# TheCacophonyProject/classifier-pipeline

Measured on AMD Instinct MI355X. Metric: CPTV frames/s end-to-end (track+classify) at 160x120, higher is better.
Workload: dtype u16/i32 track stage (f32 normalise, f64 gates); f32 crop/tile; f32 CNN (stride-1 3x3 convs of stages 2-4 (+ the stride-2 one): two fp16 planes per operand rounded to nearest (11 + 11 significand bits), power-of-two range scaling, 3 fp16 MFMAs per K step, device-side rerun in the exact split if an ac

## Files before the change

### classifier-pipeline_amd/csrc/cpx_cnn_bf3.hip

```cpp
#include <hip/hip_runtime.h>

#include <algorithm>
#include <cstdlib>
#include <type_traits>

#include "cpx_conv_layout_core.h"
#include "cpx_kernels.h"

namespace cpx {

namespace {

typedef float f32x16 __attribute__((ext_vector_type(16)));
typedef __bf16 bf16x8 __attribute__((ext_vector_type(8)));
typedef __bf16 bf16x2 __attribute__((ext_vector_type(2)));
typedef unsigned u32x4 __attribute__((ext_vector_type(4)));
typedef float f32x4 __attribute__((ext_vector_type(4)));

__device__ __forceinline__ unsigned pack2(float a, float b) {
  bf16x2 v = {(__bf16)a, (__bf16)b};
  return __builtin_bit_cast(unsigned, v);
}
template <typename T>
__device__ __forceinline__ const T* at_off(const T* base, unsigned bytes) {
// ... 1938 lines not shown
    return launch_bf3w(a, im, w, s);
  }
  if (a.Cout / a.groups == 32) return launch_bf3_t<1, 1, NB_S2, TW_S2, CT_S2>(a, w, s);
  if (a.Cout / a.groups == 64) return launch_bf3_t<NTN_S3, 1, NB_S3, TW_S3, CT_S3>(a, w, s);
  if (flat_pays(a, 32, 4 * NB_S4, 256)) {
    if (a.planes == 2 && a.half && a.sc_in && a.sc_planes && conv_shortcut_planes_layer(a, a.sc_cin / a.groups) && !a.residual &&
        a.sc_stride >= 1 && a.sc_xscale > 0.0f && (a.sc_H - 1) / a.sc_stride + 1 == a.Ho && (a.sc_W - 1) / a.sc_stride + 1 == a.Wo &&
        (long long)a.sc_H * a.sc_W * a.sc_cin < (1ll << 31))
      return launch_bf3flat_t<2, 256, 2, true, 256, true>(a, w + im.half / 16, s);
    return with_math(a, im, w, [&](auto pl, auto h, const uint4* wi) {
      return launch_bf3flat_t<2, 256, decltype(pl)::value, decltype(h)::value>(a, wi, s);
    });
  }
  return with_math(a, im, w, [&](auto pl, auto h, const uint4* wi) {
    return launch_bf3_t<NTN_S4, 1, NB_S4, 32, CT_S4, false, decltype(pl)::value, decltype(h)::value>(a, wi, s);
  });
}

bool conv_block32_supported(const ConvArgs& a, const ConvArgs& b) {
  const auto plain = [](const ConvArgs& c) {
    return c.ksize == 3 && c.stride == 1 && c.Cout / c.groups == 32 && c.relu && c.pad_top == 1 && c.pad_left == 1 && !c.out_planes &&
           !c.in_planes;
  };
  if (!(plain(a) && plain(b) && a.in_scale && a.in_shift && !a.residual && !a.sc_in && !b.in_scale && !b.out_scale &&
        a.Cout == b.Cin && b.Cin == b.Cout && a.groups == b.groups && a.H == b.H && a.W == b.W && a.N == b.N && a.ovf != nullptr))
    return false;
  if (a.Cin / a.groups == 8)
    return b.residual == nullptr && b.sc_in == a.in && b.sc_w != nullptr && b.sc_cin == a.Cin && b.sc_stride == 1 && b.sc_H == a.H &&
           b.sc_W == a.W;
  return a.Cin == a.Cout && b.residual == a.in && b.sc_in == nullptr;
}
int launch_conv_block32(const ConvArgs& a_in, const ConvArgs& b_in, const void* wimg_a, const void* wimg_b, hipStream_t s) {
  ConvArgs a = a_in, b = b_in;
  if (!conv_block32_supported(a, b)) return -2;
  if ((long long)a.H * a.W >= (1 << 24)) return -3;
  const WeightImages ia = images_of(a), ib = images_of(b);
  if (ia.half == WeightImages::absent || ib.half == WeightImages::absent) return -2;
  a.w_scale = conv_bf3_weight_scales(a, wimg_a);
  a.w_unscale = a.w_scale + a.Cout;
  b.w_scale = conv_bf3_weight_scales(b, wimg_b);
  b.w_unscale = b.w_scale + b.Cout;
  const uint4* wa = reinterpret_cast<const uint4*>(wimg_a) + ia.half / 16;
  const uint4* wb = reinterpret_cast<const uint4*>(wimg_b) + ib.half / 16;
  TileDiv td{};
  if (const int rc = fill_tiles(td, (a.W + W_TW - 1) / W_TW, (a.H + W_TH - 1) / W_TH, a.N, 1, TILES_PERSISTENT)) return rc;
  const bool c8 = a.Cin / a.groups == 8;
  static const bool split_roles = [] {
    const char* e = std::getenv("CPX_BLOCK32_SPLIT");
    return e == nullptr || std::atoi(e) != 0;
  }();
  if (!c8 && split_roles) return launch_conv_block32s(a, b, wa, wb, s);
  const bool c1 = c8 && a.c1_in != nullptr;
  if (c1 && !(a.groups == 2 && a.c1_w != nullptr && a.c1_b != nullptr)) return -2;
  const size_t lds = c8 ? (size_t)(B_R0 + B8_WIMG + B_WIMG) * 16 + 256 + (size_t)2 * B8_NPXP * 16 + (c1 ? (size_t)(B_C1W + 2 * B_C1C) * 4 : 0)
                        : (size_t)(B_R0 + 2 * B_WIMG) * 16 + 256;
  static bool lds_ready[64], lds_ready8[64], lds_ready1[64];
  if (c1 ? !cpx_dyn_lds_ready(reinterpret_cast<const void*>(conv_block32_kernel<true, true>), lds_ready1, 160 * 1024 - 1024)
      : c8 ? !cpx_dyn_lds_ready(reinterpret_cast<const void*>(conv_block32_kernel<true>), lds_ready8, 160 * 1024 - 1024)
           : !cpx_dyn_lds_ready(reinterpret_cast<const void*>(conv_block32_kernel<false>), lds_ready, 160 * 1024 - 1024))
    return -1;
  const int cus = cpx_device_cus();
  if (cus == 0) return -1;
  const char* e = std::getenv("CPX_BLOCK32_GRID");
  const int gx = e ? persistent_grid_x(std::atoi(e), 1, td.total) : persistent_grid_x(cus, a.groups, td.total);
  if (c1) hipLaunchKernelGGL((conv_block32_kernel<true, true>), dim3((unsigned)gx, a.groups), dim3(512), lds, s, a, b, wa, wb, td);
  else if (c8) hipLaunchKernelGGL(conv_block32_kernel<true>, dim3((unsigned)gx, a.groups), dim3(512), lds, s, a, b, wa, wb, td);
  else hipLaunchKernelGGL(conv_block32_kernel<false>, dim3((unsigned)gx, a.groups), dim3(512), lds, s, a, b, wa, wb, td);
  return 0;
}

}
```

### classifier-pipeline_amd/csrc/cpx_cnn_blk.hip

```cpp
#include <hip/hip_runtime.h>

#include <algorithm>
#include <cstdlib>
#include <type_traits>

#include "cpx_conv_layout_core.h"
#include "cpx_kernels.h"

namespace cpx {

namespace {

typedef unsigned u32x4 __attribute__((ext_vector_type(4)));
typedef float f32x4 __attribute__((ext_vector_type(4)));
typedef _Float16 f16x2 __attribute__((ext_vector_type(2)));
typedef _Float16 f16x8 __attribute__((ext_vector_type(8)));

template <typename T>
__device__ __forceinline__ const T* at_off(const T* base, unsigned bytes) {
  return reinterpret_cast<const T*>(reinterpret_cast<const char*>(base) + bytes);
}
template <typename T>
__device__ __forceinline__ T* at_off(T* base, unsigned bytes) {
  return reinterpret_cast<T*>(reinterpret_cast<char*>(base) + bytes);
}
__device__ __forceinline__ unsigned pix_off(int y, int x, int W, int C) {
  return __umul24(__umul24((unsigned)y, (unsigned)W) + (unsigned)x, (unsigned)C);
}
__device__ __forceinline__ float relu_bits(float x) { return __int_as_float(max(__float_as_int(x), 0)); }
__device__ __forceinline__ void split_h(float a, float b, unsigned& hi, unsigned& lo) {
  f16x2 v = {(_Float16)a, (_Float16)b};
  hi = __builtin_bit_cast(unsigned, v);
  asm("v_fma_mixlo_f16 %0, %1, 1.0, -%2 op_sel:[0,0,0] op_sel_hi:[0,0,1]" : "=v"(lo) : "v"(a), "v"(hi));
  asm("v_fma_mixhi_f16 %0, %1, 1.0, -%2 op_sel:[0,0,1] op_sel_hi:[0,0,1]" : "+v"(lo) : "v"(b), "v"(hi));
}
__device__ __forceinline__ f32x4 mfma_h(u32x4 w, u32x4 x, f32x4 c) {
  return __builtin_amdgcn_mfma_f32_16x16x32_f16(__builtin_bit_cast(f16x8, w), __builtin_bit_cast(f16x8, x), c, 0, 0, 0);
}
__device__ __forceinline__ unsigned pk_max_u16(unsigned x, unsigned y) {
  unsigned r;
  asm("v_pk_max_u16 %0, %1, %2" : "=v"(r) : "v"(x), "v"(y));
  return r;
}
__device__ __forceinline__ int med3(int x, int lo, int hi) {
  int r;
  asm("v_med3_i32 %0, %1, %2, %3" : "=v"(r) : "v"(x), "v"(lo), "s"(hi));
  return r;
}
template <int I, int N, typename F>
__device__ __forceinline__ void static_for(F&& f) {
  if constexpr (I < N) {
    f(std::integral_constant<int, I>{});
    static_for<I + 1, N>(f);
  }
}
struct BlkTiles {
  unsigned long long m_tx, m_ty;
  int tiles_x, tiles_y, total;
};
__device__ __forceinline__ int div_magic(int n, unsigned long long m) { return (int)(((unsigned long long)n * m) >> 42); }

constexpr int K_T = 16;
constexpr int K_PP = 20, K_PNPX = 400;
constexpr int K_PNPXP = 402;
constexpr int K_MP = 18;
constexpr int K_MNPXP = 326;
constexpr int K_PBUF = 2 * 2 * K_PNPXP * 2;
constexpr int K_MBUF = 2 * 2 * K_MNPXP * 2;
constexpr int K_CT = 512;
constexpr int K_NP = 7;
constexpr int K_PPI = K_CT / 8;
constexpr int K_WROW = 2 * 3 * 4 * 32;
constexpr int K_WIMG = 3 * K_WROW;
constexpr size_t K_LDS = (size_t)(K_PBUF + 2 * K_MBUF) * 16;

__global__ __launch_bounds__(K_CT) __attribute__((amdgpu_waves_per_eu(2, 2))) void conv_block32s_kernel(ConvArgs a, ConvArgs b, const uint4* __restrict__ wa, const uint4* __restrict__ wb, BlkTiles td) {
  if (*a.ovf != 0) return;
  extern __shared__ __attribute__((aligned(16))) uint4 lds4[];
  uint4* s_P = lds4;
  uint4* s_M = lds4 + K_PBUF;
  const int tid = threadIdx.x, lane = tid & 63, wave = tid >> 6, i16 = lane & 15, q = lane >> 4;
  const bool is_a = wave < 4;
  const int ct = wave & 1, hh = (wave >> 1) & 1;
  const int g = blockIdx.y;
  const int C = b.Cout, H = a.H, W = a.W;

  u32x4 Wr[9][2];
  {
    const u32x4* wg = reinterpret_cast<const u32x4*>(is_a ? wa : wb) + (size_t)g * K_WIMG + q * 32 + ct * 16 + i16;
#pragma unroll
    for (int ky = 0; ky < 3; ++ky)
#pragma unroll
      for (int kx = 0; kx < 3; ++kx)
#pragma unroll
        for (int p = 0; p < 2; ++p) Wr[ky * 3 + kx][p] = wg[ky * K_WROW + (p * 3 + kx) * 128];
  }
  const int ch_l = g * 32 + ct * 16 + 4 * q;
  f32x4 os, ob, rs = {1.0f, 1.0f, 1.0f, 1.0f};
  if (is_a) {
    os = *reinterpret_cast<const f32x4*>(a.w_unscale + ch_l) * (a.act_unscale * b.act_scale);
    if (a.out_scale) os *= *reinterpret_cast<const f32x4*>(a.out_scale + ch_l);
    ob = f32x4{0.0f, 0.0f, 0.0f, 0.0f};
    if (a.out_shift) ob = *reinterpret_cast<const f32x4*>(a.out_shift + ch_l) * b.act_scale;
  } else {
    rs = *reinterpret_cast<const f32x4*>(b.w_scale + ch_l) * b.act_scale;
    os = *reinterpret_cast<const f32x4*>(b.w_unscale + ch_l) * b.act_unscale;
    ob = f32x4{0.0f, 0.0f, 0.0f, 0.0f};
    if (b.out_shift) ob = *reinterpret_cast<const f32x4*>(b.out_shift + ch_l);
  }

  const int per_xcd = (td.total + 7) >> 3;
  auto tile_of = [&](int t) { return (t & 7) * per_xcd + (t >> 3); };
  auto get_tile = [&](int j, int& n_, int& oy_, int& ox_) {
    const int t = (int)blockIdx.x + j * (int)gridDim.x;
    if (t >= 8 * per_xcd) return false;
    int tile = tile_of(t);
    if (tile >= td.total) return false;
    int qd = div_magic(tile, td.m_tx);
    ox_ = (tile - qd * td.tiles_x) * K_T;
    tile = qd;
    qd = div_magic(tile, td.m_ty);
    oy_ = (tile - qd * td.tiles_y) * K_T;
    n_ = qd;
    return true;
  };

  u32x4 pre_p[K_NP];
  const int q8 = tid & 7;
  int ipos[K_NP];
#pragma unroll
  for (int i = 0; i < K_NP; ++i) {
    const int px = min((tid >> 3) + K_PPI * i, K_PNPX - 1);
    const int py = px / K_PP;
    ipos[i] = (py << 8) | (px - py * K_PP);
  }
  const unsigned st_base = (unsigned)((((q8 >> 2) * K_PNPXP + (tid >> 3)) * 4 + (q8 & 3)) * 8);
  f32x4 psc, psh;
  psc = *reinterpret_cast<const f32x4*>(a.in_scale + g * 32 + 4 * q8) * a.act_scale;
  psh = *reinterpret_cast<const f32x4*>(a.in_shift + g * 32 + 4 * q8) * a.act_scale;
  const unsigned coff0 = (unsigned)(g * 32 + 4 * q8);
  const int Hm1 = H - 1, Wm1 = W - 1;
  auto issue_item = [&](const int i, const int n_, const int oy_, const int ox_) __attribute__((always_inline)) {
    const float* in_n = a.in + (size_t)n_ * H * W * a.Cin;
    const int iy = oy_ - 2 + (ipos[i] >> 8), ix = ox_ - 2 + (ipos[i] & 0xFF);
    const int cy = med3(iy, 0, Hm1), cx = med3(ix, 0, Wm1);
    pre_p[i] = *reinterpret_cast<const u32x4*>(at_off(in_n, (pix_off(cy, cx, W, a.Cin) + coff0) << 2));
  };
  unsigned hmax = 0u;
  auto convert_item = [&](const int i, const int oy_, const int ox_) __attribute__((always_inline)) {
    float v[4];
#pragma unroll
    for (int j = 0; j < 4; ++j) v[j] = fmaxf(__fmaf_rn(__uint_as_float(pre_p[i][j]), psc[j], psh[j]), 0.0f);
    const int iy = oy_ - 2 + (ipos[i] >> 8), ix = ox_ - 2 + (ipos[i] & 0xFF);
    const bool inside = (unsigned)iy < (unsigned)H && (unsigned)ix < (unsigned)W;
#pragma unroll
    for (int j = 0; j < 4; ++j) v[j] = inside ? v[j] : 0.0f;
    unsigned h0, h1, l0, l1;
    split_h(v[0], v[1], h0, l0);
    split_h(v[2], v[3], h1, l1);
    hmax = pk_max_u16(pk_max_u16(hmax, h0), h1);
    pre_p[i] = u32x4{h0, h1, l0, l1};
  };
  auto store_item = [&](const int i) __attribute__((always_inline)) {
    if (i == K_NP - 1 && tid >= K_PNPX * 8 - (K_NP - 1) * K_CT) return;
    const u32x4 v = pre_p[i];
    unsigned char* sp = reinterpret_cast<unsigned char*>(s_P) + st_base;
    *reinterpret_cast<uint2*>(sp + i * (K_PPI * 32)) = make_uint2(v[0], v[1]);
    *reinterpret_cast<uint2*>(sp + 2 * K_PNPXP * 32 + i * (K_PPI * 32)) = make_uint2(v[2], v[3]);
  };

  f32x4 acc[11];
  constexpr int AHEAD = 3, RING = 4;

  auto conv_a = [&](auto&& between) __attribute__((always_inline)) {
    const uint4* pb = s_P + ((q >> 1) * K_PNPXP + (9 * hh) * K_PP + i16) * 2 + (q & 1);
#pragma unroll
    for (int o = 0; o < 11; ++o) acc[o] = f32x4{0.0f, 0.0f, 0.0f, 0.0f};
    u32x4 xh[RING], xl[RING];
    auto frag = [&](auto sc) __attribute__((always_inline)) {
      constexpr int s = decltype(sc)::value, kx = s / 11, i = s - 11 * kx, bf = s % RING;
      xh[bf] = __builtin_bit_cast(u32x4, pb[(i * K_PP + kx) * 2]);
      xl[bf] = __builtin_bit_cast(u32x4, pb[4 * K_PNPXP + (i * K_PP + kx) * 2]);
    };
    static_for<0, AHEAD>(frag);
    static_for<0, 33>([&](auto sc) __attribute__((always_inline)) {
      constexpr int s = decltype(sc)::value, kx = s / 11, i = s - 11 * kx, bf = s % RING;
      if constexpr (s + AHEAD < 33) frag(std::integral_constant<int, s + AHEAD>{});
      static_for<0, 3>([&](auto pc) __attribute__((always_inline)) {
        constexpr int pr = decltype(pc)::value;
        static_for<0, 3>([&](auto rc) __attribute__((always_inline)) {
          constexpr int r = decltype(rc)::value, o = i - r;
          if constexpr (o >= 0 && o < 9) {
            if constexpr (pr == 0) acc[o] = mfma_h(Wr[r * 3 + kx][1], xh[bf], acc[o]);
            if constexpr (pr == 1) acc[o] = mfma_h(Wr[r * 3 + kx][0], xl[bf], acc[o]);
            if constexpr (pr == 2) acc[o] = mfma_h(Wr[r * 3 + kx][0], xh[bf], acc[o]);
          }
        });
      });
      between(sc);
      __builtin_amdgcn_sched_barrier(0);
    });
    int eb[2];
#pragma unroll
    for (int k = 0; k < 2; ++k) {
      const int e = min((hh ? 16 * k : 32) + i16, 35);
      eb[k] = ((q >> 1) * K_PNPXP + (e >> 1) * K_PP + 16 + (e & 1)) * 2 + (q & 1);
    }
    static_for<0, 9>([&](auto tc) __attribute__((always_inline)) {
      constexpr int tp = decltype(tc)::value, kx = tp / 3, ky = tp - 3 * kx;
      u32x4 eh[2], el[2];
#pragma unroll
      for (int k = 0; k < 2; ++k) {
        if (k == 0 || hh) {
          eh[k] = __builtin_bit_cast(u32x4, s_P[eb[k] + (ky * K_PP + kx) * 2]);
          el[k] = __builtin_bit_cast(u32x4, s_P[4 * K_PNPXP + eb[k] + (ky * K_PP + kx) * 2]);
        }
      }
#pragma unroll
      for (int k = 0; k < 2; ++k) {
        if (k == 0 || hh) {
          acc[9 + k] = mfma_h(Wr[ky * 3 + kx][1], eh[k], acc[9 + k]);
          acc[9 + k] = mfma_h(Wr[ky * 3 + kx][0], el[k], acc[9 + k]);
          acc[9 + k] = mfma_h(Wr[ky * 3 + kx][0], eh[k], acc[9 + k]);
        }
      }
      between(std::integral_constant<int, 33 + tp>{});
    });
  };
  auto mid_put = [&](const int par, const int oy_, const int ox_, const f32x4 accv, const int mrow, const int mcol, const bool valid) __attribute__((always_inline)) {
    unsigned char* mb = reinterpret_cast<unsigned char*>(s_M + par * K_MBUF);
    f32x4 v;
#pragma unroll
    for (int j = 0; j < 4; ++j) v[j] = fmaxf(__fmaf_rn(accv[j], os[j], ob[j]), 0.0f);
    const bool inside = (unsigned)(oy_ - 1 + mrow) < (unsigned)H && (unsigned)(ox_ - 1 + mcol) < (unsigned)W;
#pragma unroll
    for (int j = 0; j < 4; ++j) v[j] = inside ? v[j] : 0.0f;
    unsigned h0, h1, l0, l1;
    split_h(v[0], v[1], h0, l0);
    split_h(v[2], v[3], h1, l1);
    hmax = pk_max_u16(pk_max_u16(hmax, h0), h1);
    const unsigned off = (unsigned)(((ct * K_MNPXP + mrow * K_MP + mcol) * 4 + q) * 8);
    if (valid) {
      *reinterpret_cast<uint2*>(mb + off) = make_uint2(h0, h1);
      *reinterpret_cast<uint2*>(mb + off + 2 * K_MNPXP * 32) = make_uint2(l0, l1);
    }
  };
  auto mid_row = [&](const int par, const int oy_, const int ox_, const int o) __attribute__((always_inline)) {
    mid_put(par, oy_, ox_, acc[o], 9 * hh + o, i16, true);
  };
  auto mid_edges = [&](const int par, const int oy_, const int ox_) __attribute__((always_inline)) {
#pragma unroll
    for (int k = 0; k < 2; ++k) {
      if (k == 0 || hh) {
        const int e = (hh ? 16 * k : 32) + i16;
        mid_put(par, oy_, ox_, acc[9 + k], min(e, 35) >> 1, 16 + (e & 1), e < 36);
      }
    }
  };
  auto conv_b = [&](const int par, auto&& between) __attribute__((always_inline)) {
    const uint4* mbp = s_M + par * K_MBUF + ((q >> 1) * K_MNPXP + (8 * hh) * K_MP + i16) * 2 + (q & 1);
#pragma unroll
    for (int o = 0; o < 8; ++o) acc[o] = acc[o] * rs;
    u32x4 xh[RING], xl[RING];
    auto frag = [&](auto sc) __attribute__((always_inline)) {
      constexpr int s = decltype(sc)::value, kx = s / 10, i = s - 10 * kx, bf = s % RING;
      xh[bf] = __builtin_bit_cast(u32x4, mbp[(i * K_MP + kx) * 2]);
      xl[bf] = __builtin_bit_cast(u32x4, mbp[4 * K_MNPXP + (i * K_MP + kx) * 2]);
    };
    static_for<0, AHEAD>(frag);
    static_for<0, 30>([&](auto sc) __attribute__((always_inline)) {
      constexpr int s = decltype(sc)::value, kx = s / 10, i = s - 10 * kx, bf = s % RING;
      if constexpr (s + AHEAD < 30) frag(std::integral_constant<int, s + AHEAD>{});
      static_for<0, 3>([&](auto pc) __attribute__((always_inline)) {
        constexpr int pr = decltype(pc)::value;
        static_for<0, 3>([&](auto rc) __attribute__((always_inline)) {
          constexpr int r = decltype(rc)::value, o = i - r;
          if constexpr (o >= 0 && o < 8) {
            if constexpr (pr == 0) acc[o] = mfma_h(Wr[r * 3 + kx][1], xh[bf], acc[o]);
            if constexpr (pr == 1) acc[o] = mfma_h(Wr[r * 3 + kx][0], xl[bf], acc[o]);
            if constexpr (pr == 2) acc[o] = mfma_h(Wr[r * 3 + kx][0], xh[bf], acc[o]);
          }
        });
      });
      between(sc);
      __builtin_amdgcn_sched_barrier(0);
    });
  };
  auto preload_res = [&](const int n_, const int oy_, const int ox_) __attribute__((always_inline)) {
    const float* res_n = b.residual + (size_t)n_ * H * W * C;
    const int ox = min(ox_ + i16, Wm1);
#pragma unroll
    for (int o = 0; o < 8; ++o) {
      const int oy = min(oy_ + 8 * hh + o, Hm1);
      acc[o] = *reinterpret_cast<const f32x4*>(at_off(res_n, (pix_off(oy, ox, W, C) + (unsigned)ch_l) << 2));
    }
  };
  auto out_row = [&](const int n_, const int oy_, const int ox_, const int o) __attribute__((always_inline)) {
    float* out_n = b.out + (size_t)n_ * H * W * C;
    const int ox = min(ox_ + i16, Wm1);
    const int oy = oy_ + 8 * hh + o;
    const unsigned off = (pix_off(min(oy, Hm1), ox, W, C) + (unsigned)ch_l) << 2;
    f32x4 v;
#pragma unroll
    for (int j = 0; j < 4; ++j) v[j] = __fmaf_rn(acc[o][j], os[j], ob[j]);
    v.x = relu_bits(v.x); v.y = relu_bits(v.y); v.z = relu_bits(v.z); v.w = relu_bits(v.w);
    if (ox_ + i16 < W && oy < H) *reinterpret_cast<f32x4*>(at_off(out_n, off)) = v;
  };

  int n0 = 0, oy0 = 0, ox0 = 0, n1 = 0, oy1 = 0, ox1 = 0, n2 = 0, oy2 = 0, ox2 = 0;
  bool v0 = false;
  bool v1 = get_tile(0, n1, oy1, ox1);
  if (!v1) return;
  bool v2 = get_tile(1, n2, oy2, ox2);
#pragma unroll
  for (int i = 0; i < K_NP; ++i) issue_item(i, n1, oy1, ox1);
#pragma unroll
  for (int i = 0; i < K_NP; ++i) {
    convert_item(i, oy1, ox1);
    store_item(i);
  }
  __syncthreads();
  for (int k = -1;; ++k) {
    const int oyc = v2 ? oy2 : oy1, oxc = v2 ? ox2 : ox1;
    auto stage = [&](const int i) __attribute__((always_inline)) {
      issue_item(i, v2 ? n2 : n1, oyc, oxc);
    };
    if (is_a) {
      if (v1) {
        conv_a([&](auto sc) __attribute__((always_inline)) {
          constexpr int s = decltype(sc)::value;
          if constexpr (s % 5 == 2 && s / 5 < K_NP) stage(s / 5);
          if constexpr (s >= 25 && s <= 32) mid_row((k + 1) & 1, oy1, ox1, s - 25);
        });
        mid_row((k + 1) & 1, oy1, ox1, 8);
        mid_edges((k + 1) & 1, oy1, ox1);
      } else {
#pragma unroll
        for (int i = 0; i < K_NP; ++i) stage(i);
      }
    } else {
      if (v0) {
        conv_b(k & 1, [&](auto sc) __attribute__((always_inline)) {
          constexpr int s = decltype(sc)::value;
          if constexpr (s % 4 == 1 && s / 4 < K_NP) stage(s / 4);
          if constexpr (s >= 23 && s <= 29) out_row(n0, oy0, ox0, s - 23);
        });
        out_row(n0, oy0, ox0, 7);
      } else {
#pragma unroll
        for (int i = 0; i < K_NP; ++i) stage(i);
      }
      if (v1) preload_res(n1, oy1, ox1);
    }
    __syncthreads();
    if (v2) {
#pragma unroll
      for (int i = 0; i < K_NP; ++i) {
        if (is_a) {
          convert_item(i, oy2, ox2);
          store_item(i);
        } else {
          convert_item(i, oy2, ox2);
          store_item(i);
        }
      }
    }
    if (!v1) break;
    __syncthreads();
    n0 = n1; oy0 = oy1; ox0 = ox1; v0 = v1;
    n1 = n2; oy1 = oy2; ox1 = ox2; v1 = v2;
    v2 = v1 && get_tile(k + 3, n2, oy2, ox2);
  }
  if ((hmax & 0xFFFFu) >= 0x7C00u || (hmax >> 16) >= 0x7C00u) atomicOr(a.ovf, 1);
}


}

int launch_conv_block32s(const ConvArgs& a, const ConvArgs& b, const void* wa, const void* wb, hipStream_t s) {
  BlkTiles td{};
  if (const int rc = fill_tiles(td, (a.W + K_T - 1) / K_T, (a.H + K_T - 1) / K_T, a.N, TILES_PERSISTENT)) return rc;
  static bool lds_ready[64];
  if (!cpx_dyn_lds_ready(reinterpret_cast<const void*>(conv_block32s_kernel), lds_ready, 160 * 1024 - 1024)) return -1;
  const int cus = cpx_device_cus();
  if (cus == 0) return -1;
  const char* e = std::getenv("CPX_BLOCK32_GRID");
  const int gx = e ? persistent_grid_x(std::atoi(e), 1, td.total) : persistent_grid_x(cus, a.groups, td.total);
  hipLaunchKernelGGL(conv_block32s_kernel, dim3((unsigned)gx, a.groups), dim3(K_CT), K_LDS, s, a, b, reinterpret_cast<const uint4*>(wa),
                     reinterpret_cast<const uint4*>(wb), td);
  return 0;
}

}
```

### classifier-pipeline_amd/csrc/cpx_conv_layout_core.h

```cpp
#pragma once
#include <stddef.h>

#include <algorithm>

namespace cpx {

struct ConvShape { int groups, cin_g, cout_g, ksize, stride; };
template <class Args>
ConvShape conv_shape_of(const Args& a) {
  if (a.groups < 1 || a.Cin % a.groups || a.Cout % a.groups) return ConvShape{};
  return ConvShape{a.groups, a.Cin / a.groups, a.Cout / a.groups, a.ksize, a.stride};
}

enum class ConvClass { Unsupported, Plain, Flat, Wide, C8, Stride2Rw, Rw3 };

inline ConvClass conv_class(const ConvShape& s) {
  if (s.ksize != 3) return ConvClass::Unsupported;
  if (s.stride == 3 && s.cin_g == 64 && s.cout_g == 128) return ConvClass::Rw3;
  if (s.stride == 2 && s.cin_g == 32 && s.cout_g == 64) return ConvClass::Stride2Rw;
  if (s.stride == 1 && s.cin_g == 8 && s.cout_g == 32) return ConvClass::C8;
  const bool c32_64 = s.cout_g == 32 || s.cout_g == 64;
  if (s.stride == 1 && (s.cin_g == 32 || s.cin_g == 64) && c32_64) return ConvClass::Wide;
  if (s.cin_g < 16 || s.cin_g % 16) return ConvClass::Unsupported;
  if ((s.stride == 1 && s.cout_g == 128) || (s.stride == 2 && s.cout_g == 64)) return ConvClass::Flat;
// ... 12 lines not shown
  static constexpr size_t absent = ~(size_t)0;
  static constexpr size_t C8_HALF_ENTRIES = 3 * 2 * 4 * 32;
  ConvClass cls = ConvClass::Unsupported;
  int chunk = 0;
  size_t planes3 = absent, planes2 = absent, half = absent, scales = absent, rw_half = absent, bytes = 0;

  static WeightImages of(const ConvShape& s) {
    WeightImages l;
    l.cls = conv_class(s);
    if (l.cls == ConvClass::Unsupported) return l;
    const auto put = [&l](size_t& image, size_t size) { image = l.bytes; l.bytes += size; };
    const size_t row = (size_t)s.cout_g * 16;
    const size_t scales = ((size_t)2 * s.groups * s.cout_g * sizeof(float) + 15) / 16 * 16;
    if (l.cls == ConvClass::C8) {
      put(l.planes3, (size_t)s.groups * 30 * row);
      put(l.half, (size_t)s.groups * C8_HALF_ENTRIES * 16);
      put(l.scales, scales);
      return l;
    }
    l.chunk = l.cls == ConvClass::Wide || l.cls == ConvClass::Rw3 ? 32 : 16;
    const auto image = [&](int planes) { return (size_t)s.groups * (s.cin_g / l.chunk) * (9 * l.chunk / 8 * planes) * row; };
    if (l.cls != ConvClass::Rw3) put(l.planes3, image(3));
    if (l.cls == ConvClass::Plain) return l;
    if (l.cls != ConvClass::Rw3) put(l.planes2, image(2));
    put(l.half, image(2));
    put(l.scales, scales);
    if (l.cls == ConvClass::Stride2Rw) put(l.rw_half, image(2));
    return l;
  }
};

constexpr int TILE_AXIS_LIMIT = 4096;
constexpr long long TILES_PER_LAUNCH = 1ll << 22;
constexpr long long TILES_PERSISTENT = (1ll << 22) - 8;
inline unsigned long long tile_magic(int d) { return (1ull << 42) / (unsigned long long)d + 1; }

template <class Tiles>
int fill_tiles(Tiles& td, int tiles_x, int tiles_y, long long n, long long limit) {
  if (tiles_x < 1 || tiles_y < 1 || tiles_x >= TILE_AXIS_LIMIT || tiles_y >= TILE_AXIS_LIMIT) return -3;
  const long long total = (long long)tiles_x * tiles_y * n;
  if (total >= limit) return -3;
  td.tiles_x = tiles_x, td.m_tx = tile_magic(tiles_x);
  td.tiles_y = tiles_y, td.m_ty = tile_magic(tiles_y);
  td.total = (int)total;
  return 0;
}
template <class Tiles>
int fill_tiles(Tiles& td, int tiles_x, int tiles_y, long long n, int nsplit, long long limit) {
  if (nsplit < 1 || nsplit >= TILE_AXIS_LIMIT) return -3;
  td.nsplit = nsplit, td.m_nsplit = tile_magic(nsplit);
  return fill_tiles(td, tiles_x, tiles_y, n * nsplit, limit);
}

inline int persistent_grid_x(int cus, int ny, long long tiles) {
  const int gx = std::max(8, cus / std::max(ny, 1) / 8 * 8);
  return (int)std::min<long long>(gx, (tiles + 7) / 8 * 8);
}

}
```

### classifier-pipeline_amd/csrc/cpx_kernels.h

```cpp
#pragma once
#include <hip/hip_runtime.h>
#include <stddef.h>
#include <stdint.h>

#include "cpx.h"

#ifndef CPX_TRACK_THREADS
#define CPX_TRACK_THREADS 768
#endif
#ifndef CPX_TRACK_CHUNKS
#define CPX_TRACK_CHUNKS 7
#endif
#ifndef CPX_TRACK_LDS_COMPONENTS
#define CPX_TRACK_LDS_COMPONENTS 256
#endif
#ifndef CPX_TRACK_MIN_WAVES_PER_SIMD
#define CPX_TRACK_MIN_WAVES_PER_SIMD 6
#endif

namespace cpx {

typedef cpx_component Component;
typedef cpx_frame_info FrameInfo;

// ... 139 lines not shown
  int Ho, Wo, pad_top, pad_left;
  const float* in;
  float* out;
  const float* weights;
  const float* in_scale;
  const float* in_shift;
  const float* out_scale;
  const float* out_shift;
  const float* residual;
  const float* sc_in;
  const float* sc_w;
  const float* sc_bias;
  int sc_H, sc_W, sc_cin, sc_stride;
  const void* sc_planes;
  float sc_xscale;
  const float* c1_in;
  const float* c1_w;
  const float* c1_b;
  int planes;
  int half;
  float act_scale, act_unscale;
  const float* w_scale;
  const float* w_unscale;
  int* ovf;
  const int* guard;
  int out_planes, in_planes;
  float out_act_scale;
};
struct HeadArgs {
  int N, HW, C, L;
  int n_hidden, activation;
  int hidden_sizes[CPX_HEAD_MAX_HIDDEN];
  const float* in;
  const float* bn_scale;
  const float* bn_shift;
  const float* hidden_w[CPX_HEAD_MAX_HIDDEN];
  const float* hidden_b[CPX_HEAD_MAX_HIDDEN];
  const float* dense_w;
  const float* dense_b;
  float* logits;
  float* probs;
};
int launch_conv(const ConvArgs& a, hipStream_t s);
bool conv_bf3_supported(const ConvArgs& a);
size_t conv_bf3_weight_bytes(const ConvArgs& a);
bool conv_bf3_two_planes(const ConvArgs& a);
bool conv_bf3_can_store_planes(const ConvArgs& a);
bool conv_bf3_can_load_planes(const ConvArgs& a);
void launch_split_weights(const ConvArgs& a, void* wimg, hipStream_t s);
int launch_conv_bf3(const ConvArgs& a, const void* wimg, hipStream_t s);
bool conv_block32_supported(const ConvArgs& a, const ConvArgs& b);
int launch_conv_block32(const ConvArgs& a, const ConvArgs& b, const void* wimg_a, const void* wimg_b, hipStream_t s);
int launch_conv_block32s(const ConvArgs& a, const ConvArgs& b, const void* wa, const void* wb, hipStream_t s);
int conv_rw_kind(const ConvArgs& a);
bool conv_rw_layer(const ConvArgs& a);
int launch_conv_rw(const ConvArgs& a, const void* wimg, hipStream_t s);
bool conv_shortcut_planes_layer(const ConvArgs& second, int sc_cin_g);
size_t conv_shortcut_image_bytes(int groups, int cin_g, int cout_g);
void launch_split_shortcut(const float* sc_w, void* img, int groups, int cin_g, int cout_g, const float* w_scale, float factor,
                           hipStream_t s);
const float* conv_bf3_weight_scales(const ConvArgs& a, const void* wimg);
void launch_head(const HeadArgs& a, hipStream_t s);
void launch_count_overflow(int* ovf, int n_words, hipStream_t s);

struct CptvArgs {
  int W, H;
  const unsigned char* payload;
  const long long* frame_offsets;
  const int* bit_widths;
  const int* clip_offsets;
  uint16_t* frames_out;
};
int launch_cptv_unpack(const CptvArgs& a, int B, hipStream_t s);

struct CptvInflateArgs {
  int B;
  const unsigned char* in;
  const cpx_cptv_file* files;
  unsigned char* out;
  cpx_cptv_frame_slot* slots;
  unsigned char* header;
  cpx_cptv_file_result* results;
};
int launch_cptv_inflate(const CptvInflateArgs& a, hipStream_t s);

struct CptvGatherArgs {
  const cpx_cptv_frame_slot* slots;
  const long long* slot_offsets;
  const int* clip_offsets;
  long long* frame_offsets;
  int* bit_widths;
  cpx_cptv_frame_slot* slots_out;
};
int launch_cptv_gather(const CptvGatherArgs& a, int B, hipStream_t s);

struct ThumbArgs {
  int W, H, chain_cap;
  int max_w, max_h;
  const uint16_t* frames;
  const int32_t* labels;
  const cpx_frame_info* info;
  const cpx_region_ref* refs;
  cpx_thumb_stat* out;
};
int launch_thumb(const ThumbArgs& a, int n_refs, hipStream_t s);

// ... 129 lines not shown
```

Baseline: 3.115 million.

## Add twin-resident 256-thread fused block8 kernel with c1 conv prefetch overlap

Adds a new 256-thread conv_block8t kernel for the c8 block that also folds in the preceding c1 conv. Its LDS is kept under half a CU so two workgroups can be resident per CU, and the persistent grid is doubled to match. The next tile's c1 inputs are loaded and converted while the current tile's MFMAs run, with weights held in registers. It is enabled by default behind an env switch and adds a large new kernel with register-pressure and correctness risk.

```diff
diff --git a/classifier-pipeline_amd/csrc/cpx_cnn_bf3.hip b/classifier-pipeline_amd/csrc/cpx_cnn_bf3.hip
--- a/classifier-pipeline_amd/csrc/cpx_cnn_bf3.hip
+++ b/classifier-pipeline_amd/csrc/cpx_cnn_bf3.hip
@@ -2014,6 +2014,11 @@
   if (!c8 && split_roles) return launch_conv_block32s(a, b, wa, wb, s);
   const bool c1 = c8 && a.c1_in != nullptr;
   if (c1 && !(a.groups == 2 && a.c1_w != nullptr && a.c1_b != nullptr)) return -2;
+  static const bool twin = [] {
+    const char* e = std::getenv("CPX_BLOCK8_TWIN");
+    return e == nullptr || std::atoi(e) != 0;
+  }();
+  if (c1 && twin) return launch_conv_block8t(a, b, wa, wb, s);
   const size_t lds = c8 ? (size_t)(B_R0 + B8_WIMG + B_WIMG) * 16 + 256 + (size_t)2 * B8_NPXP * 16 + (c1 ? (size_t)(B_C1W + 2 * B_C1C) * 4 : 0)
                         : (size_t)(B_R0 + 2 * B_WIMG) * 16 + 256;
   static bool lds_ready[64], lds_ready8[64], lds_ready1[64];
diff --git a/classifier-pipeline_amd/csrc/cpx_cnn_blk.hip b/classifier-pipeline_amd/csrc/cpx_cnn_blk.hip
--- a/classifier-pipeline_amd/csrc/cpx_cnn_blk.hip
+++ b/classifier-pipeline_amd/csrc/cpx_cnn_blk.hip
@@ -374,6 +374,336 @@
   if ((hmax & 0xFFFFu) >= 0x7C00u || (hmax >> 16) >= 0x7C00u) atomicOr(a.ovf, 1);
 }
 
+constexpr int T_CT = 256;
+constexpr int T_PNPXP = K_PNPX + 2;
+constexpr int T_WA = 3 * 2 * 4 * 32;
+constexpr int T_C1W = 96;
+constexpr int T_C1C = 256 * 8;
+constexpr int T_NGRP = 21;
+constexpr int T_PAR = 16 + 8 * 4;
+constexpr size_t T_LDS = (size_t)(K_MBUF + 2 * T_PNPXP + T_PAR) * 16 + (size_t)(T_C1W + 2 * T_C1C) * 4;
+static_assert(T_LDS <= 79 * 1024, "two workgroups of conv_block8t_kernel fit a CU's 160 KB of LDS");
+static_assert(T_WA == (int)WeightImages::C8_HALF_ENTRIES, "conv_block8t_kernel and the layout agree on the tap-quad image");
+
+__global__ __launch_bounds__(T_CT) __attribute__((amdgpu_waves_per_eu(2, 2))) void conv_block8t_kernel(ConvArgs a, ConvArgs b, const uint4* __restrict__ wa, const uint4* __restrict__ wb, BlkTiles td) {
+  if (*a.ovf != 0) return;
+  extern __shared__ __attribute__((aligned(16))) uint4 lds4[];
+  uint4* s_M = lds4;
+  uint4* s_px = lds4 + K_MBUF;
+  f32x4* s_bn = reinterpret_cast<f32x4*>(s_px + 2 * T_PNPXP);
+  f32x4* s_ep = s_bn + 16;
+  float* s_c1w = reinterpret_cast<float*>(s_bn + T_PAR);
+  float* s_c1c = s_c1w + T_C1W;
+  const int tid = threadIdx.x, lane = tid & 63, wave = __builtin_amdgcn_readfirstlane(tid >> 6), i16 = lane & 15, q = lane >> 4;
+  const int ct = wave & 1, hh = wave >> 1;
+  const int g = blockIdx.y;
+  const int C = b.Cout, H = a.H, W = a.W;
+
+  if (tid < 8) {
+    reinterpret_cast<float*>(s_bn)[tid] = a.in_scale[g * 8 + tid] * a.act_scale;
+    reinterpret_cast<float*>(s_bn)[8 + tid] = a.in_shift[g * 8 + tid] * a.act_scale;
+  }
+  if (tid < 2) reinterpret_cast<u32x4*>(s_px)[tid * T_PNPXP + K_PNPX] = u32x4{0u, 0u, 0u, 0u};
+  if (tid < 80) s_c1w[tid] = tid < 72 ? a.c1_w[g * 72 + tid] : a.c1_b[g * 8 + tid - 72];
+
+  const int per_xcd = (td.total + 7) >> 3;
+  auto tile_of = [&](int t) { return (t & 7) * per_xcd + (t >> 3); };
+  int n, oy0, ox0;
+  auto decode = [&](int tile) {
+    int qd = div_magic(tile, td.m_tx);
+    ox0 = (tile - qd * td.tiles_x) * K_T;
+    tile = qd;
+    qd = div_magic(tile, td.m_ty);
+    oy0 = (tile - qd * td.tiles_y) * K_T;
+    n = qd;
+  };
+  int t = blockIdx.x;
+  while (t < 8 * per_xcd && tile_of(t) >= td.total) t += gridDim.x;
+  if (t >= 8 * per_xcd) return;
+  decode(tile_of(t));
+
+  float c1_raw[2][9];
+  auto c1_pixel = [&](const int k, int& py, int& pxx) __attribute__((always_inline)) {
+    int t8 = tid + T_CT * k;
+    asm volatile("" : "+v"(t8));
+    const int px = min(t8, K_PNPX - 1);
+    py = (int)(__umul24((unsigned)px, 3277u) >> 16);
+    pxx = __mul24(py, -K_PP) + px;
+  };
+  auto issue_c1 = [&](const int k) __attribute__((always_inline)) {
+    int py, pxx;
+    c1_pixel(k, py, pxx);
+    const float* in_n = a.c1_in + (size_t)n * H * W * a.groups + g;
+#pragma unroll
+    for (int ky = 0; ky < 3; ++ky)
+#pragma unroll
+      for (int kx = 0; kx < 3; ++kx) {
+        const int cy = min(max(oy0 - 3 + py + ky, 0), H - 1), cx = min(max(ox0 - 3 + pxx + kx, 0), W - 1);
+        c1_raw[k][ky * 3 + kx] = *at_off(in_n, (unsigned)((cy * W + cx) * a.groups) << 2);
+      }
+  };
+  issue_c1(0);
+  issue_c1(1);
+
+  u32x4 Wb[9][2], Wa[3][2];
+  {
+    const u32x4* wgb = reinterpret_cast<const u32x4*>(wb) + (size_t)g * K_WIMG + q * 32 + ct * 16 + i16;
+#pragma unroll
+    for (int ky = 0; ky < 3; ++ky)
+#pragma unroll
+      for (int kx = 0; kx < 3; ++kx)
+#pragma unroll
+        for (int p = 0; p < 2; ++p) Wb[ky * 3 + kx][p] = wgb[ky * K_WROW + (p * 3 + kx) * 128];
+    const u32x4* wga = reinterpret_cast<const u32x4*>(wa) + (size_t)g * T_WA + q * 32 + ct * 16 + i16;
+#pragma unroll
+    for (int t4 = 0; t4 < 3; ++t4)
+#pragma unroll
+      for (int p = 0; p < 2; ++p) Wa[t4][p] = wga[(t4 * 2 + p) * 128];
+  }
+  float wsc[2];
+  {
+    const float ss = b.w_scale[g * 32 + 16 * ct + i16] * b.act_scale;
+#pragma unroll
+    for (int k = 0; k < 2; ++k) wsc[k] = b.sc_w[((size_t)g * 8 + q + 4 * k) * 32 + 16 * ct + i16] * ss;
+  }
+  const int ch_l = g * 32 + ct * 16 + 4 * q;
+  const f32x4* ep = s_ep + (ct * 4 + q) * 4;
+  if (hh == 0 && i16 == 0) {
+  f32x4 os_a, ob_a, os_b, ob_b;
+  os_a = *reinterpret_cast<const f32x4*>(a.w_unscale + ch_l) * (a.act_unscale * b.act_scale);
+  if (a.out_scale) os_a *= *reinterpret_cast<const f32x4*>(a.out_scale + ch_l);
+  ob_a = f32x4{0.0f, 0.0f, 0.0f, 0.0f};
+  if (a.out_shift) ob_a = *reinterpret_cast<const f32x4*>(a.out_shift + ch_l) * b.act_scale;
+  os_b = *reinterpret_cast<const f32x4*>(b.w_unscale + ch_l) * b.act_unscale;
+  ob_b = f32x4{0.0f, 0.0f, 0.0f, 0.0f};
+  if (b.out_shift) ob_b = *reinterpret_cast<const f32x4*>(b.out_shift + ch_l);
+  if (b.sc_bias) ob_b += *reinterpret_cast<const f32x4*>(b.sc_bias + ch_l);
+  f32x4* epw = s_ep + (ct * 4 + q) * 4;
+  epw[0] = os_a; epw[1] = ob_a; epw[2] = os_b; epw[3] = ob_b;
+  }
+  __syncthreads();
+
+  unsigned hmax = 0u;
+  float acc8[8];
+  auto convert_c1 = [&](const int k, const int part, const int py0, const int px0, const bool interior, const int buf) __attribute__((always_inline)) {
+    int py, pxx;
+    c1_pixel(k, py, pxx);
+    if (part == 0) {
+#pragma unroll
+      for (int c = 0; c < 8; ++c) acc8[c] = 0.0f;
+    }
+#pragma unroll
+    for (int tp = 3 * part; tp < 3 * part + 3; ++tp) {
+      float v = c1_raw[k][tp];
+      if (!interior) {
+        const int ky = tp / 3, kx = tp - 3 * ky;
+        v = ((unsigned)(py0 - 1 + py + ky) < (unsigned)H && (unsigned)(px0 - 1 + pxx + kx) < (unsigned)W) ? v : 0.0f;
+      }
+      const f32x4 w0 = *reinterpret_cast<const f32x4*>(s_c1w + tp * 8), w1 = *reinterpret_cast<const f32x4*>(s_c1w + tp * 8 + 4);
+#pragma unroll
+      for (int c = 0; c < 4; ++c) {
+        acc8[c] = __fmaf_rn(v, w0[c], acc8[c]);
+        acc8[4 + c] = __fmaf_rn(v, w1[c], acc8[4 + c]);
+      }
+    }
+    if (part < 2) return;
+    const f32x4 bs0 = *reinterpret_cast<const f32x4*>(s_c1w + 72), bs1 = *reinterpret_cast<const f32x4*>(s_c1w + 76);
+    f32x4 x0, x1;
+#pragma unroll
+    for (int c = 0; c < 4; ++c) {
+      x0[c] = acc8[c] + bs0[c];
+      x1[c] = acc8[4 + c] + bs1[c];
+    }
+    int tpx = tid + T_CT * k;
+    asm volatile("" : "+v"(tpx));
+    const bool mine = tpx < K_PNPX;
+    if ((unsigned)(py - 2) < 16u && (unsigned)(pxx - 2) < 16u && mine) {
+      f32x4* cc = reinterpret_cast<f32x4*>(s_c1c + buf * T_C1C + ((py - 2) * 16 + (pxx - 2)) * 8);
+      cc[0] = x0;
+      cc[1] = x1;
+    }
+    f32x4 y0 = __builtin_elementwise_fma(x0, s_bn[0], s_bn[2]), y1 = __builtin_elementwise_fma(x1, s_bn[1], s_bn[3]);
+    const bool inside = interior || ((unsigned)(py0 + py) < (unsigned)H && (unsigned)(px0 + pxx) < (unsigned)W);
+#pragma unroll
+    for (int j = 0; j < 4; ++j) {
+      y0[j] = inside ? fmaxf(y0[j], 0.0f) : 0.0f;
+      y1[j] = inside ? fmaxf(y1[j], 0.0f) : 0.0f;
+    }
+    unsigned h0, h1, h2, h3, l0, l1, l2, l3;
+    split_h(y0[0], y0[1], h0, l0);
+    split_h(y0[2], y0[3], h1, l1);
+    split_h(y1[0], y1[1], h2, l2);
+    split_h(y1[2], y1[3], h3, l3);
+    hmax = pk_max_u16(pk_max_u16(pk_max_u16(pk_max_u16(hmax, h0), h1), h2), h3);
+    if (mine) {
+      reinterpret_cast<u32x4*>(s_px)[tpx] = u32x4{h0, h1, h2, h3};
+      reinterpret_cast<u32x4*>(s_px)[T_PNPXP + tpx] = u32x4{l0, l1, l2, l3};
+    }
+  };
+  auto tile_interior = [&]() { return oy0 - 3 >= 0 && oy0 + 16 + 3 <= H && ox0 - 3 >= 0 && ox0 + 16 + 3 <= W; };
+  int cbuf = 0;
+  {
+    const bool interior = tile_interior();
+#pragma unroll
+    for (int k = 0; k < 2; ++k)
+#pragma unroll
+      for (int part = 0; part < 3; ++part) convert_c1(k, part, oy0 - 2, ox0 - 2, interior, 0);
+  }
+
+  int toff[3];
+#pragma unroll
+  for (int t4 = 0; t4 < 3; ++t4) {
+    const int tap = 4 * t4 + q;
+    const int ky = (tap * 11) >> 5;
+    toff[t4] = ky * K_PP + (tap - 3 * ky);
+  }
+  const bool tap_zero = q != 0;
+  const int ngrp = hh ? T_NGRP - 11 : 11;
+  constexpr int AHEAD = 3, RING = 4;
+  constexpr int GB = 3, NBT = 4;
+
+  for (;;) {
+    const int n_cur = n, oy_cur = oy0, ox_cur = ox0;
+    const bool interior_cur = tile_interior();
+    bool more = false, interior_next = false;
+    __syncthreads();
+    {
+      f32x4 acc1[GB];
+      u32x4 xa[2][GB][2];
+      int abase[GB];
+      auto batch_base = [&](const int bt) __attribute__((always_inline)) {
+        int pb = 16 * (11 * hh + GB * bt) + i16;
+        asm volatile("" : "+v"(pb));
+#pragma unroll
+        for (int j = 0; j < GB; ++j) {
+          const int p = min(pb + 16 * j, K_MP * K_MP - 1);
+          const int my = (int)(__umul24((unsigned)p, 3641u) >> 16), mx = p - my * K_MP;
+          abase[j] = my * K_PP + mx;
+        }
+      };
+      auto frag_a = [&](const int bt, const int t4, const int bf) __attribute__((always_inline)) {
+#pragma unroll
+        for (int j = 0; j < GB; ++j) {
+          if (GB * bt + j < ngrp) {
+            const int e = (t4 == 2 && tap_zero) ? K_PNPX : abase[j] + toff[t4];
+            xa[bf][j][0] = __builtin_bit_cast(u32x4, s_px[e]);
+            xa[bf][j][1] = __builtin_bit_cast(u32x4, s_px[T_PNPXP + e]);
+          }
+        }
+      };
+      auto mid_epilogue = [&](const int bt) __attribute__((always_inline)) {
+        int pb = 16 * (11 * hh + GB * bt) + i16;
+        asm volatile("" : "+v"(pb));
+#pragma unroll
+        for (int j = 0; j < GB; ++j) {
+          const int p = pb + 16 * j;
+          if (GB * bt + j < ngrp && p < K_MP * K_MP) {
+            f32x4 v = acc1[j] * ep[0] + ep[1];
+            v.x = relu_bits(v.x); v.y = relu_bits(v.y); v.z = relu_bits(v.z); v.w = relu_bits(v.w);
+            unsigned h0, h1, l0, l1;
+            split_h(v.x, v.y, h0, l0);
+            split_h(v.z, v.w, h1, l1);
+            hmax = pk_max_u16(pk_max_u16(hmax, h0), h1);
+            if (!interior_cur) {
+              asm volatile("");
+              const int my = (int)(__umul24((unsigned)p, 3641u) >> 16), mx = p - my * K_MP;
+              const bool inside = (unsigned)(oy_cur - 1 + my) < (unsigned)H && (unsigned)(ox_cur - 1 + mx) < (unsigned)W;
+              h0 = inside ? h0 : 0u; h1 = inside ? h1 : 0u; l0 = inside ? l0 : 0u; l1 = inside ? l1 : 0u;
+            }
+            uint2* sp2 = reinterpret_cast<uint2*>(s_M) + (ct * K_MNPXP + p) * 4 + q;
+            sp2[0] = make_uint2(h0, h1);
+            sp2[(2 * K_MNPXP) * 4] = make_uint2(l0, l1);
+          }
+        }
+      };
+      batch_base(0);
+      frag_a(0, 0, 0);
+      static_for<0, 3 * NBT>([&](auto uc) __attribute__((always_inline)) {
+        constexpr int u = decltype(uc)::value, bt = u / 3, t4 = u - 3 * bt, bf = u & 1;
+        if constexpr (t4 == 0) {
+#pragma unroll
+          for (int j = 0; j < GB; ++j) acc1[j] = f32x4{0.0f, 0.0f, 0.0f, 0.0f};
+        }
+        if constexpr (t4 < 2) frag_a(bt, t4 + 1, bf ^ 1);
+        else if constexpr (bt + 1 < NBT) {
+          batch_base(bt + 1);
+          frag_a(bt + 1, 0, bf ^ 1);
+        }
+        static_for<0, 3>([&](auto pc) __attribute__((always_inline)) {
+          constexpr int pr = decltype(pc)::value;
+#pragma unroll
+          for (int j = 0; j < GB; ++j) {
+            if (GB * bt + j < ngrp) {
+              if constexpr (pr == 0) acc1[j] = mfma_h(Wa[t4][1], xa[bf][j][0], acc1[j]);
+              if constexpr (pr == 1) acc1[j] = mfma_h(Wa[t4][0], xa[bf][j][1], acc1[j]);
+              if constexpr (pr == 2) acc1[j] = mfma_h(Wa[t4][0], xa[bf][j][0], acc1[j]);
+            }
+          }
+        });
+        if constexpr (u == 0) {
+          t += gridDim.x;
+          more = t < 8 * per_xcd && tile_of(t) < td.total;
+          if (more) decode(tile_of(t));
+          interior_next = tile_interior();
+        }
+        if constexpr (u == 1 || u == 2) {
+          if (more) issue_c1(u - 1);
+        }
+        if constexpr (t4 == 2) mid_epilogue(bt);
+      });
+    }
+    __syncthreads();
+    {
+      f32x4 acc[8];
+#pragma unroll
+      for (int o = 0; o < 8; ++o) acc[o] = f32x4{0.0f, 0.0f, 0.0f, 0.0f};
+      const uint4* mbp = s_M + ((q >> 1) * K_MNPXP + (8 * hh) * K_MP + i16) * 2 + (q & 1);
+      float* out_n = b.out + (size_t)n_cur * H * W * C;
+      const float* ccb = s_c1c + cbuf * T_C1C + ((8 * hh) * 16 + i16) * 8 + q;
+      auto out_row = [&](const int o) __attribute__((always_inline)) {
+#pragma unroll
+        for (int k = 0; k < 2; ++k) acc[o] = __builtin_amdgcn_mfma_f32_16x16x4f32(wsc[k], ccb[o * 128 + 4 * k], acc[o], 0, 0, 0);
+        const int oy = oy_cur + 8 * hh + o, ox = ox_cur + i16;
+        const unsigned off = (pix_off(min(oy, H - 1), min(ox, W - 1), W, C) + (unsigned)ch_l) << 2;
+        f32x4 v = acc[o] * ep[2];
+        v += ep[3];
+        v.x = relu_bits(v.x); v.y = relu_bits(v.y); v.z = relu_bits(v.z); v.w = relu_bits(v.w);
+        if (oy < H && ox < W) *reinterpret_cast<f32x4*>(at_off(out_n, off)) = v;
+      };
+      u32x4 xh[RING], xl[RING];
+      auto frag = [&](auto sc) __attribute__((always_inline)) {
+        constexpr int s = decltype(sc)::value, i = s / 3, kx = s - 3 * i, bf = s % RING;
+        xh[bf] = __builtin_bit_cast(u32x4, mbp[(i * K_MP + kx) * 2]);
+        xl[bf] = __builtin_bit_cast(u32x4, mbp[4 * K_MNPXP + (i * K_MP + kx) * 2]);
+      };
+      static_for<0, AHEAD>(frag);
+      static_for<0, 30>([&](auto sc) __attribute__((always_inline)) {
+        constexpr int s = decltype(sc)::value, i = s / 3, kx = s - 3 * i, bf = s % RING;
+        if constexpr (s + AHEAD < 30) frag(std::integral_constant<int, s + AHEAD>{});
+        static_for<0, 3>([&](auto pc) __attribute__((always_inline)) {
+          constexpr int pr = decltype(pc)::value;
+          static_for<0, 3>([&](auto rc) __attribute__((always_inline)) {
+            constexpr int r = decltype(rc)::value, o = i - r;
+            if constexpr (o >= 0 && o < 8) {
+              if constexpr (pr == 0) acc[o] = mfma_h(Wb[r * 3 + kx][1], xh[bf], acc[o]);
+              if constexpr (pr == 1) acc[o] = mfma_h(Wb[r * 3 + kx][0], xl[bf], acc[o]);
+              if constexpr (pr == 2) acc[o] = mfma_h(Wb[r * 3 + kx][0], xh[bf], acc[o]);
+            }
+          });
+        });
+        if constexpr (s >= 1 && s <= 6) {
+          if (more) convert_c1((s - 1) / 3, (s - 1) % 3, oy0 - 2, ox0 - 2, interior_next, cbuf ^ 1);
+        }
+        if constexpr (s >= 9 && s % 3 == 0) out_row(s / 3 - 3);
+        __builtin_amdgcn_sched_barrier(0);
+      });
+      out_row(7);
+    }
+    if (!more) break;
+    cbuf ^= 1;
+  }
+  if ((hmax & 0xFFFFu) >= 0x7C00u || (hmax >> 16) >= 0x7C00u) atomicOr(a.ovf, 1);
+}
 
 }
 
@@ -391,4 +721,19 @@
   return 0;
 }
 
-}
+int launch_conv_block8t(const ConvArgs& a, const ConvArgs& b, const void* wa, const void* wb, hipStream_t s) {
+  if (a.Cin / a.groups != 8 || a.c1_in == nullptr || a.c1_w == nullptr || a.c1_b == nullptr || a.groups != 2) return -2;
+  BlkTiles td{};
+  if (const int rc = fill_tiles(td, (a.W + K_T - 1) / K_T, (a.H + K_T - 1) / K_T, a.N, TILES_PERSISTENT)) return rc;
+  static bool lds_ready[64];
+  if (!cpx_dyn_lds_ready(reinterpret_cast<const void*>(conv_block8t_kernel), lds_ready, 79 * 1024)) return -1;
+  const int cus = cpx_device_cus();
+  if (cus == 0) return -1;
+  const char* e = std::getenv("CPX_BLOCK32_GRID");
+  const int gx = e ? persistent_grid_x(std::atoi(e), 1, td.total) : persistent_grid_x(cus, a.groups, td.total, 2);
+  hipLaunchKernelGGL(conv_block8t_kernel, dim3((unsigned)gx, a.groups), dim3(T_CT), T_LDS, s, a, b, reinterpret_cast<const uint4*>(wa),
+                     reinterpret_cast<const uint4*>(wb), td);
+  return 0;
+}
+
+}
diff --git a/classifier-pipeline_amd/csrc/cpx_conv_layout_core.h b/classifier-pipeline_amd/csrc/cpx_conv_layout_core.h
--- a/classifier-pipeline_amd/csrc/cpx_conv_layout_core.h
+++ b/classifier-pipeline_amd/csrc/cpx_conv_layout_core.h
@@ -88,9 +88,10 @@
   return fill_tiles(td, tiles_x, tiles_y, n * nsplit, limit);
 }
 
-inline int persistent_grid_x(int cus, int ny, long long tiles) {
-  const int gx = std::max(8, cus / std::max(ny, 1) / 8 * 8);
+inline int persistent_grid_x(int cus, int ny, long long tiles, int per_cu) {
+  const int gx = std::max(8, cus * std::max(per_cu, 1) / std::max(ny, 1) / 8 * 8);
   return (int)std::min<long long>(gx, (tiles + 7) / 8 * 8);
 }
+inline int persistent_grid_x(int cus, int ny, long long tiles) { return persistent_grid_x(cus, ny, tiles, 1); }
 
 }
diff --git a/classifier-pipeline_amd/csrc/cpx_kernels.h b/classifier-pipeline_amd/csrc/cpx_kernels.h
--- a/classifier-pipeline_amd/csrc/cpx_kernels.h
+++ b/classifier-pipeline_amd/csrc/cpx_kernels.h
@@ -215,6 +215,7 @@
 bool conv_block32_supported(const ConvArgs& a, const ConvArgs& b);
 int launch_conv_block32(const ConvArgs& a, const ConvArgs& b, const void* wimg_a, const void* wimg_b, hipStream_t s);
 int launch_conv_block32s(const ConvArgs& a, const ConvArgs& b, const void* wa, const void* wb, hipStream_t s);
+int launch_conv_block8t(const ConvArgs& a, const ConvArgs& b, const void* wa, const void* wb, hipStream_t s);
 int conv_rw_kind(const ConvArgs& a);
 bool conv_rw_layer(const ConvArgs& a);
 int launch_conv_rw(const ConvArgs& a, const void* wimg, hipStream_t s);
```

New measurement: 3.124 million (median of 3 runs). Within noise of the previous version (+0.3%).

## Walk tiles row-wise right-to-left and carry mid-layer halo between adjacent tiles

Applied to the files above, without the earlier changes.

Adds a row-walk tile schedule in which each persistent workgroup processes a full row of tiles from right to left. When consecutive tiles are horizontally adjacent, the overlapping intermediate-activation halo columns are copied between LDS ring buffers instead of recomputed, so the edge-column part of the first conv is skipped. A host heuristic picks row or tile walking from the estimated per-workgroup work with an assumed carry saving, and environment variables can override both. The cost is coarser load balancing with row units, plus extra LDS copies and branching in the fused block kernel.

```diff
diff --git a/classifier-pipeline_amd/csrc/cpx_cnn_blk.hip b/classifier-pipeline_amd/csrc/cpx_cnn_blk.hip
--- a/classifier-pipeline_amd/csrc/cpx_cnn_blk.hip
+++ b/classifier-pipeline_amd/csrc/cpx_cnn_blk.hip
@@ -54,12 +54,6 @@
     static_for<I + 1, N>(f);
   }
 }
-struct BlkTiles {
-  unsigned long long m_tx, m_ty;
-  int tiles_x, tiles_y, total;
-};
-__device__ __forceinline__ int div_magic(int n, unsigned long long m) { return (int)(((unsigned long long)n * m) >> 42); }
-
 constexpr int K_T = 16;
 constexpr int K_PP = 20, K_PNPX = 400;
 constexpr int K_PNPXP = 402;
@@ -74,7 +68,7 @@
 constexpr int K_WIMG = 3 * K_WROW;
 constexpr size_t K_LDS = (size_t)(K_PBUF + 2 * K_MBUF) * 16;
 
-__global__ __launch_bounds__(K_CT) __attribute__((amdgpu_waves_per_eu(2, 2))) void conv_block32s_kernel(ConvArgs a, ConvArgs b, const uint4* __restrict__ wa, const uint4* __restrict__ wb, BlkTiles td) {
+__global__ __launch_bounds__(K_CT) __attribute__((amdgpu_waves_per_eu(2, 2))) void conv_block32s_kernel(ConvArgs a, ConvArgs b, const uint4* __restrict__ wa, const uint4* __restrict__ wb, BlkTiles td, int carry_on) {
   if (*a.ovf != 0) return;
   extern __shared__ __attribute__((aligned(16))) uint4 lds4[];
   uint4* s_P = lds4;
@@ -109,19 +103,11 @@
     if (b.out_shift) ob = *reinterpret_cast<const f32x4*>(b.out_shift + ch_l);
   }
 
-  const int per_xcd = (td.total + 7) >> 3;
-  auto tile_of = [&](int t) { return (t & 7) * per_xcd + (t >> 3); };
   auto get_tile = [&](int j, int& n_, int& oy_, int& ox_) {
-    const int t = (int)blockIdx.x + j * (int)gridDim.x;
-    if (t >= 8 * per_xcd) return false;
-    int tile = tile_of(t);
-    if (tile >= td.total) return false;
-    int qd = div_magic(tile, td.m_tx);
-    ox_ = (tile - qd * td.tiles_x) * K_T;
-    tile = qd;
-    qd = div_magic(tile, td.m_ty);
-    oy_ = (tile - qd * td.tiles_y) * K_T;
-    n_ = qd;
+    int ty, tx;
+    if (!walk_tile(td, (int)blockIdx.x, (int)gridDim.x, j, n_, ty, tx)) return false;
+    oy_ = ty * K_T;
+    ox_ = tx * K_T;
     return true;
   };
 
@@ -172,7 +158,7 @@
   f32x4 acc[11];
   constexpr int AHEAD = 3, RING = 4;
 
-  auto conv_a = [&](auto&& between) __attribute__((always_inline)) {
+  auto conv_a = [&](const bool carry, auto&& between) __attribute__((always_inline)) {
     const uint4* pb = s_P + ((q >> 1) * K_PNPXP + (9 * hh) * K_PP + i16) * 2 + (q & 1);
 #pragma unroll
     for (int o = 0; o < 11; ++o) acc[o] = f32x4{0.0f, 0.0f, 0.0f, 0.0f};
@@ -200,6 +186,7 @@
       between(sc);
       __builtin_amdgcn_sched_barrier(0);
     });
+    if (carry) return;
     int eb[2];
 #pragma unroll
     for (int k = 0; k < 2; ++k) {
@@ -256,6 +243,18 @@
         mid_put(par, oy_, ox_, acc[9 + k], min(e, 35) >> 1, 16 + (e & 1), e < 36);
       }
     }
+  };
+  auto carry_idx = [&](const int e) { return (((e >> 2) / K_MP) * K_MNPXP + ((e >> 2) % K_MP) * K_MP) * 2 + (e & 3); };
+  u32x4 cc[2];
+  auto carry_load = [&](const int par) __attribute__((always_inline)) {
+    const uint4* src = s_M + (par ^ 1) * K_MBUF;
+    cc[0] = __builtin_bit_cast(u32x4, src[carry_idx(tid)]);
+    if (tid < 32) cc[1] = __builtin_bit_cast(u32x4, src[carry_idx(256 + tid)]);
+  };
+  auto carry_store = [&](const int par) __attribute__((always_inline)) {
+    uint4* dst = s_M + par * K_MBUF + K_T * 2;
+    dst[carry_idx(tid)] = __builtin_bit_cast(uint4, cc[0]);
+    if (tid < 32) dst[carry_idx(256 + tid)] = __builtin_bit_cast(uint4, cc[1]);
   };
   auto conv_b = [&](const int par, auto&& between) __attribute__((always_inline)) {
     const uint4* mbp = s_M + par * K_MBUF + ((q >> 1) * K_MNPXP + (8 * hh) * K_MP + i16) * 2 + (q & 1);
@@ -327,13 +326,20 @@
     };
     if (is_a) {
       if (v1) {
-        conv_a([&](auto sc) __attribute__((always_inline)) {
+        const bool carry = carry_on && v0 && n0 == n1 && oy0 == oy1 && ox1 + K_T == ox0;
+        conv_a(carry, [&](auto sc) __attribute__((always_inline)) {
           constexpr int s = decltype(sc)::value;
           if constexpr (s % 5 == 2 && s / 5 < K_NP) stage(s / 5);
+          if constexpr (s == 24) {
+            if (carry) carry_load((k + 1) & 1);
+          }
+          if constexpr (s == 27) {
+            if (carry) carry_store((k + 1) & 1);
+          }
           if constexpr (s >= 25 && s <= 32) mid_row((k + 1) & 1, oy1, ox1, s - 25);
         });
         mid_row((k + 1) & 1, oy1, ox1, 8);
-        mid_edges((k + 1) & 1, oy1, ox1);
+        if (!carry) mid_edges((k + 1) & 1, oy1, ox1);
       } else {
 #pragma unroll
         for (int i = 0; i < K_NP; ++i) stage(i);
@@ -386,8 +392,11 @@
   if (cus == 0) return -1;
   const char* e = std::getenv("CPX_BLOCK32_GRID");
   const int gx = e ? persistent_grid_x(std::atoi(e), 1, td.total) : persistent_grid_x(cus, a.groups, td.total);
+  const char* ec = std::getenv("CPX_BLOCK32_CARRY");
+  const char* ew = std::getenv("CPX_BLOCK32_WALK");
+  set_walk(td, ew ? (std::atoi(ew) ? WALK_ROWS : WALK_TILES) : choose_walk(td, gx));
   hipLaunchKernelGGL(conv_block32s_kernel, dim3((unsigned)gx, a.groups), dim3(K_CT), K_LDS, s, a, b, reinterpret_cast<const uint4*>(wa),
-                     reinterpret_cast<const uint4*>(wb), td);
+                     reinterpret_cast<const uint4*>(wb), td, ec ? (std::atoi(ec) != 0) : 1);
   return 0;
 }
 
diff --git a/classifier-pipeline_amd/csrc/cpx_conv_layout_core.h b/classifier-pipeline_amd/csrc/cpx_conv_layout_core.h
--- a/classifier-pipeline_amd/csrc/cpx_conv_layout_core.h
+++ b/classifier-pipeline_amd/csrc/cpx_conv_layout_core.h
@@ -93,4 +93,54 @@
   return (int)std::min<long long>(gx, (tiles + 7) / 8 * 8);
 }
 
+#if defined(__HIPCC__)
+#define CPX_WALK_HD __host__ __device__ __forceinline__
+#else
+#define CPX_WALK_HD inline
+#endif
+enum { WALK_TILES = 0, WALK_ROWS = 1 };
+struct BlkTiles {
+  unsigned long long m_tx, m_ty;
+  int tiles_x, tiles_y, total;
+  int walk, units;
+};
+CPX_WALK_HD int tile_div(int n, unsigned long long m) { return (int)(((unsigned long long)n * m) >> 42); }
+inline void set_walk(BlkTiles& td, int walk) {
+  td.walk = walk;
+  td.units = walk == WALK_ROWS ? td.total / td.tiles_x : td.total;
 }
+CPX_WALK_HD bool walk_tile(const BlkTiles& td, int bx, int gx, int j, int& n, int& ty, int& tx) {
+  int col = 0;
+  if (td.walk == WALK_ROWS) {
+    const int jr = tile_div(j, td.m_tx);
+    col = j - jr * td.tiles_x;
+    j = jr;
+  }
+  const int per_xcd = (td.units + 7) >> 3;
+  const int t = bx + j * gx;
+  if (t >= 8 * per_xcd) return false;
+  int unit = (t & 7) * per_xcd + (t >> 3);
+  if (unit >= td.units) return false;
+  if (td.walk == WALK_ROWS) {
+    tx = td.tiles_x - 1 - col;
+  } else {
+    const int qd = tile_div(unit, td.m_tx);
+    tx = unit - qd * td.tiles_x;
+    unit = qd;
+  }
+  n = tile_div(unit, td.m_ty);
+  ty = unit - n * td.tiles_y;
+  return true;
+}
+inline long long walk_max_tiles(const BlkTiles& td, int walk, int gx) {
+  const long long units = walk == WALK_ROWS ? td.total / td.tiles_x : td.total;
+  const long long per_xcd = (units + 7) / 8, wgs = gx / 8;
+  return (per_xcd + wgs - 1) / wgs * (walk == WALK_ROWS ? td.tiles_x : 1);
+}
+constexpr double WALK_CARRY_SAVING = 0.06;
+inline int choose_walk(const BlkTiles& td, int gx) {
+  const double rows = (double)walk_max_tiles(td, WALK_ROWS, gx) / td.tiles_x * (td.tiles_x - WALK_CARRY_SAVING * (td.tiles_x - 1));
+  return rows < (double)walk_max_tiles(td, WALK_TILES, gx) ? WALK_ROWS : WALK_TILES;
+}
+
+}
```

Measured after the change: 3.116 million before, 3.149 million after (median of 6 runs). +1.1%, better.
